# LitLeo/3m-asr-inference

Hardware: AMD Instinct MI355X
Metric: encoder frames/sec, 18Lx32e Conformer-MoE, 206-frame utterance (higher is better)
Workload: dtype f32; 1 GPU; 18-layer 32-expert fp32 (v_mfma_f32_16x16x4_f32), batch=1x206 frames per GPU, all experts local (BASELINE.json configs[1]); layers=18, experts=32, frames=206, batch_per_gpu=1, parallelism=replicas x1, streams_per_gpu=4, hip_graph=True, kernels_per_forward=267, fold_pos_proj=True, routing=balanced, route_mode=staged, packed_rows=False, fork_embed=auto

## Files before the change

### 3m-asr-inference_amd/csrc/engine.hip

```cpp
#include <assert.h>
#include <math.h>
#include <stdlib.h>
#include <string.h>

#include <functional>
#include <memory>
#include <string>
#include <unordered_map>
#include <vector>

#include "../../include/m3asr.h"
#include "common.h"
#include "kernels.h"

namespace m3 {
struct MoeWorkspace {
  int32_t* mapping; int32_t* acc; int32_t* pos; float* slab; size_t bytes;
};
MoeWorkspace carve_moe_workspace(void* base, int S, int E, int D, int F);
}

using namespace m3;

namespace {
// ... 57 lines not shown
  struct Bound {
    int B = 0, T = 0, Tp = 0, S = 0;
    const float* feat = nullptr; const int32_t* feat_len = nullptr; float* logits = nullptr;
    void* ws = nullptr; size_t ws_bytes = 0;
    float* splitk_ws = nullptr; size_t splitk_bytes = 0;
    bool a16 = false;
    bool dma = false;
    bool packed = false;
    bool xn_skipped = false;
    bool lens_in_conv1 = false;
    const float *tail_ln_g = nullptr, *tail_ln_b = nullptr; float tail_ln_eps = 0.f; float* tail_ln_out = nullptr;
    int ep_cap = 0;
    void* sstate = nullptr; int s_hist = 0, s_maxf = 0;
    bool s_slots = false;
    int fork_first = -1, fork_mid = -1, join_at = -1;
    std::shared_ptr<float> pfold;
    std::vector<Stage> stages;
    std::unordered_map<std::string, Buf> buffers;
    int n_kernels = 0;
    hipGraphExec_t graph_exec = nullptr;
    bool graph_valid = false;
    uint64_t last_use = 0;
    bool matches(int b, int t, const float* f, const int32_t* fl, const float* lg, const void* w, size_t wb, int cap,
                 const void* st = nullptr, int hist = 0, int maxf = 0, bool slots = false) const {
      return !stages.empty() && B == b && T == t && feat == f && feat_len == fl && logits == lg && ws == w && ws_bytes == wb &&
             ep_cap == cap && sstate == st && s_hist == hist && s_maxf == maxf && s_slots == slots;
    }
  };
  Bound cur;
  std::vector<Bound> parked;
  uint64_t use_clock = 0;
  int n_captures = 0;
  int ep_capacity = 0;
  hipStream_t side = nullptr;
  hipEvent_t ev_fork = nullptr, ev_join = nullptr;
  std::unordered_map<int, std::weak_ptr<float>> pfold_by_tp;
};

namespace {

struct Switches {
  int gate_index_max_rows;
  bool self_route;
  bool hfuse;
  int router_min_rows;
  bool router_xq;
  bool router_skip_xn;
  bool fused8_adapt;
};
const Switches& switches() {
  static const Switches sw = [] {
    auto num = [](const char* name, int dflt) { const char* v = getenv(name); return v ? atoi(v) : dflt; };
    Switches w;
    w.gate_index_max_rows = num("M3_GATE_INDEX_MAX_ROWS", 512);
    w.self_route = num("M3_SELF_ROUTE", 1) != 0;
    w.hfuse = num("M3_HFUSE", 1) != 0;
    w.router_min_rows = num("M3_ROUTER_MIN_ROWS", 2048);
    w.router_xq = num("M3_ROUTER_XQ", 1) != 0;
    w.router_skip_xn = num("M3_ROUTER_SKIP_XN", 0) != 0;
    w.fused8_adapt = num("M3_FUSED8_ADAPT", 0) != 0;
    return w;
  }();
  return sw;
}

bool lookup(const m3_engine* e, const std::string& name, int64_t numel, const float** out, int dtype = M3_F32) {
  auto it = e->table.find(name);
  if (it == e->table.end()) {
    set_error("engine: weight '%s' missing from the plan", name.c_str());
    return false;
  }
// ... 89 lines not shown
  return true;
}

bool load_sub(const m3_engine* e, const std::string& p, int D, int idim, SubW* s) {
  const int F2 = ((idim - 1) / 2 - 1) / 2;
  GET(s->c1w, p + "conv.0.weight_9c", 9 * (int64_t)D);
  GET(s->c1b, p + "conv.0.bias", D);
  GETW(s->c2w, p + "conv.2.weight_ohwi", 9 * (int64_t)D * D);
  GET(s->c2b, p + "conv.2.bias", D);
  return load_lin(e, p + "out.0.", D, (int64_t)D * F2, true, &s->out);
}
#undef GET
#undef GETW
#undef GETE

inline int sub_len(int t) { return ((t - 3) / 2 + 1 - 3) / 2 + 1; }

struct Carver {
  char* base; size_t off = 0;
  explicit Carver(void* b) : base((char*)b) {}
  template <typename T> T* take(size_t n) {
    T* p = (T*)(base ? base + off : nullptr);
    off += align_up(n * sizeof(T), 256);
    return p;
  }
};

struct Plan {
  int32_t* lens;
  float *c1, *c2, *x, *emb, *h1, *qkv, *pbuf, *ctx, *glu, *dw, *xn, *rl, *eall;
  void* xb;
  int32_t* moe_fs;
  unsigned char* xq; float* xq_scale;
  float* xstats;
  int32_t* gate_idx; float* gate_val;
  void* moe_ws; size_t moe_ws_bytes;
  float* splitk; size_t splitk_bytes;
  float* taps;
  float* pfold;
  int32_t *row0, *pad_of; float* xpad; void* xbpad; float* lpk;
  int32_t *ep_acc, *ep_mapping, *ep_pos, *ep_map_send, *ep_gate_recv, *ep_overflow; float *wire_a, *wire_b; int ep_cap, ep_rows;
  bool fork;
  bool hfuse;
  float *e_c1, *e_c2, *e_x, *e_h1, *e_qkv, *e_ctx, *e_glu, *e_dw, *e_xpad, *e_splitk, *e_xstats; void *e_xb, *e_xbpad;
  size_t bytes;
};

bool use_fork_embed(const m3_engine_config& c, int B, int S) { return c.fork_embed > 0 && !c.debug_taps; }
bool use_packed_rows(const m3_engine_config& c, int B) {
  if (c.packed_rows < 0 || (c.packed_rows == 0 && B <= 1)) return false;
// ... 26 lines not shown
  p.pbuf = cv.take<float>((size_t)Tp * D * (c.num_blocks + c.embed_blocks));
  p.ctx = cv.take<float>((size_t)S * D);
  p.glu = cv.take<float>((size_t)S * D);
  p.dw = cv.take<float>((size_t)S * D);
  p.xn = cv.take<float>((size_t)S * D);
  p.xq = nullptr; p.xq_scale = nullptr; p.moe_fs = nullptr;
  if (c.weight_dtype == M3_FP8) p.moe_fs = cv.take<int32_t>(64);
  if (c.weight_dtype == M3_FP8 && D == 512) {
    p.xq = cv.take<unsigned char>((size_t)S * D);
    p.xq_scale = cv.take<float>((size_t)S);
  }
  p.rl = cv.take<float>((size_t)S * Etot);
  p.eall = cv.take<float>((size_t)S * Etot * c.num_blocks);
  p.gate_idx = cv.take<int32_t>((size_t)c.num_blocks * S);
  p.gate_val = cv.take<float>((size_t)c.num_blocks * S);
  const bool ep = world > 1 || c.ep_stages > 0;
  p.ep_cap = ep ? (ep_capacity > 0 ? ep_capacity : S) : 0;
  p.ep_rows = ep ? world * (p.ep_cap + 1) : 0;
  p.moe_ws_bytes = carve_moe_workspace(nullptr, ep ? p.ep_rows : S, c.num_experts, c.attention_dim, c.hidden_units).bytes;
  p.moe_ws = cv.take<char>(p.moe_ws_bytes * (size_t)(c.debug_taps ? c.num_blocks : 1));
  p.ep_acc = p.ep_mapping = p.ep_pos = p.ep_map_send = p.ep_gate_recv = p.ep_overflow = nullptr; p.wire_a = p.wire_b = nullptr;
  if (ep) {
    p.ep_overflow = cv.take<int32_t>(64);
    p.ep_acc = cv.take<int32_t>((size_t)Etot + 1);
    p.ep_mapping = cv.take<int32_t>(S);
    p.ep_pos = cv.take<int32_t>(S);
    p.ep_map_send = cv.take<int32_t>(S);
    p.ep_gate_recv = cv.take<int32_t>(p.ep_rows);
    p.wire_a = cv.take<float>((size_t)p.ep_rows * c.attention_dim);
    p.wire_b = cv.take<float>((size_t)p.ep_rows * c.attention_dim);
// ... 361 lines not shown
    f.slices = expert_ffn_w16_slices(f.wmode, R, E, D, F);
  }
  return f;
}

static int launch_expert(const ExpertForm& f, const BlockW& w, const float* x, const MoeWorkspace& mw, int R, int E, int D, int F,
                         hipStream_t s, const float* ln_g = nullptr, const float* ln_b = nullptr, float ln_eps = 0.f,
                         const void* xq = nullptr, const float* xq_scale = nullptr, int32_t* fs_dev = nullptr) {
  if (f.wmode >= 2)
    return launch_expert_ffn_w8a8(x, D, mw.pos, mw.acc, R, E, D, F, w.ew1, w.es1, w.eb1, w.ew2, w.es2, 1, w.h_scale, mw.slab, s,
                                  xq, xq_scale, fs_dev);
  if (f.wmode == 1) return launch_expert_ffn_bf16w(x, D, mw.pos, mw.acc, R, E, D, F, w.ew1, w.eb1, w.ew2, 1, mw.slab, s);
  return launch_expert_ffn_f32(x, D, mw.pos, mw.acc, R, E, D, F, w.ew1, w.eb1, w.ew2, 1, mw.slab, ln_g, ln_b, ln_eps, s);
}

static void add_moe_local_expert(m3_engine* e, const MoeLayer& m, const MoeRoute& r, const ExpertForm& f, const Plan& pl) {
  const bool norm = r.norm_in_expert();
  const float* xin = norm ? m.x : m.xn;
  const bool self_route = r.gate == GateForm::InExpert;
  const void* xq = r.use_xq ? pl.xq : nullptr; const float* xqs = r.use_xq ? pl.xq_scale : nullptr;
  int32_t* fs = r.fs_dev ? pl.moe_fs : nullptr;
  add_stage(e, m.pfx + "moe_local.expert", f.launches, [=](hipStream_t s) {
    const BlockW& w = *m.w;
    const float* ln_g = norm ? w.n_ff.g : nullptr; const float* ln_b = norm ? w.n_ff.b : nullptr; const float ln_eps = norm ? m.eps : 0.f;
    if (self_route)
      return launch_expert_route_ffn_f32(xin, m.D, m.rl, m.live_len, m.live_rpb, m.S, m.E, m.D, m.F, w.ew1, w.eb1, w.ew2, 1, w.eb2,
                                         m.mw.slab, m.gidx, m.gval, m.mw.mapping, m.mw.acc, m.mw.pos, s, ln_g, ln_b, ln_eps);
    return launch_expert(f, w, xin, m.mw, m.S, m.E, m.D, m.F, s, ln_g, ln_b, ln_eps, xq, xqs, fs);
  }, stage_info(f.kernel, 1, -1.0, 4.0 * m.D * m.F * m.S));
}

static void add_moe_local_combine(m3_engine* e, const MoeLayer& m, const MoeRoute& r, const ExpertForm& f, const Plan& pl) {
  const bool self_route = r.gate == GateForm::InExpert;
  const int32_t* cmap = self_route ? nullptr : m.mw.mapping;
  const float* cb2 = self_route ? nullptr : m.w->eb2;
  const int32_t* fs = r.fs_dev ? pl.moe_fs : nullptr;
  const double S = m.S, D = m.D;
  add_stage(e, m.pfx + "moe_local.combine", 1, [=](hipStream_t s) {
    const BlockW& w = *m.w;
    return launch_moe_combine(f.rows, fs ? 4 : f.slices, cmap, m.gidx, m.gv, cb2, m.x, 0.5f, w.n_final.g, w.n_final.b, m.eps, m.x,
                              m.S, m.D, s, m.xb_out, m.xstats_out, fs);
  }, stage_info("moe_combine_kernel", 1, S * D * 4 * (f.slices + 2) + (m.xb_out ? 2.0 * S * D : 0.0), S * D * (f.slices + 10)));
}

static void add_moe_ep(m3_engine* e, const MoeLayer& m, const MoeRoute& r, const Plan& pl) {
  const int S = m.S, E = m.E, Etot = m.Etot, D = m.D, F = m.F, world = m.world;
  const int cap = pl.ep_cap, R = pl.ep_rows;
// ... 307 lines not shown
  if (!engine) return;
  if (engine->ev_fork) (void)hipEventDestroy(engine->ev_fork);
  if (engine->ev_join) (void)hipEventDestroy(engine->ev_join);
  if (engine->side) (void)hipStreamDestroy(engine->side);
  if (engine->cur.graph_exec) (void)hipGraphExecDestroy(engine->cur.graph_exec);
  for (auto& b : engine->parked)
    if (b.graph_exec) (void)hipGraphExecDestroy(b.graph_exec);
  delete engine;
}

size_t m3_engine_workspace_size(const m3_engine* engine, int B, int T) {
  if (!engine || B <= 0 || T < 7) return 0;
  return make_plan(engine->cfg, nullptr, B, T, engine->ep_capacity).bytes;
}

static int prepare_impl(m3_engine* e, const float* feat, const int32_t* feat_len, int B, int T, float* logits,
                        void* workspace, size_t workspace_bytes, void* sstate, int s_hist, int s_maxf, bool s_slots = false) {
  M3_REQUIRE(e && feat && feat_len && logits && workspace, "engine_prepare: null argument");
  M3_REQUIRE(B > 0 && T >= 7, "engine_prepare: need B > 0 and T >= 7 frames (got B=%d T=%d)", B, T);
  const m3_engine_config& c = e->cfg;
  const int Tp = sub_len(T);
  M3_REQUIRE(Tp < e->pe_rows, "engine_prepare: T'=%d exceeds the positional table (%lld rows)", Tp,
             (long long)e->pe_rows);
  if (int rc = init_expert_ffn_kernels()) return rc;
  if (int rc = init_expert_ffn_bf16_kernels()) return rc;
  if (int rc = init_expert_ffn_w8_kernels()) return rc;
  if (int rc = init_gemm_bf16_tiled_kernels()) return rc;
  if (int rc = init_expert_ffn_f32_tiled_kernels()) return rc;
  if (int rc = init_expert_ffn_fused_fp8_kernels()) return rc;
  if (int rc = init_gemm_f32_tiled_kernels()) return rc;
// ... 16 lines not shown
          if (e->parked[i].last_use < e->parked[lru].last_use) lru = i;
        if (e->parked[lru].graph_exec) (void)hipGraphExecDestroy(e->parked[lru].graph_exec);
        e->parked.erase(e->parked.begin() + lru);
      }
      e->parked.push_back(std::move(e->cur));
    } else if (e->cur.graph_exec) {
      (void)hipGraphExecDestroy(e->cur.graph_exec);
    }
    e->cur = m3_engine::Bound();
  }
  for (size_t i = 0; i < e->parked.size(); ++i)
    if (e->parked[i].matches(B, T, feat, feat_len, logits, workspace, workspace_bytes, e->ep_capacity, sstate, s_hist, s_maxf, s_slots)) {
      e->cur = std::move(e->parked[i]);
      e->parked.erase(e->parked.begin() + i);
      e->cur.last_use = ++e->use_clock;
      return (int)e->cur.stages.size();
    }
  e->cur.last_use = ++e->use_clock;
  e->cur.B = B; e->cur.T = T; e->cur.Tp = Tp; e->cur.S = B * Tp;
  e->cur.feat = feat; e->cur.feat_len = feat_len; e->cur.logits = logits; e->cur.ws = workspace; e->cur.ws_bytes = workspace_bytes;
  e->cur.ep_cap = e->ep_capacity;
  e->cur.sstate = sstate; e->cur.s_hist = s_hist; e->cur.s_maxf = s_maxf; e->cur.s_slots = s_slots;
  const bool streaming = sstate != nullptr;
  e->cur.stages.clear(); e->cur.buffers.clear(); e->cur.n_kernels = 0; e->cur.graph_valid = false; e->cur.xn_skipped = false;
  e->cur.splitk_ws = pl.splitk; e->cur.splitk_bytes = pl.splitk_bytes;
  {
    GemmParams t;
    t.M = B * Tp; t.N = c.attention_dim; t.K = c.attention_dim; t.w_bf16 = 1;
    e->cur.a16 = c.weight_dtype != M3_F32 && c.bf16_activations >= 0 && !c.debug_taps && c.embed_dim == c.attention_dim &&
                 (c.embed_linear_units % 128) == 0 && (c.hidden_units % 128) == 0 && gemm_bf16w_uses_tiled(t);
  }
  {
    GemmParams t;
    t.M = B * Tp; t.N = c.attention_dim; t.K = c.attention_dim; t.lda = c.attention_dim; t.w_bf16 = 1; t.a_bf16 = 1;
    e->cur.dma = e->cur.a16 && c.attention_dim == 128 * kXbStatParts && gemm_bf16w_uses_dma(t);
  }
  e->cur.packed = use_packed_rows(c, B);
  if (streaming) {
    e->cur.a16 = e->cur.dma = e->cur.packed = false;
// ... 120 lines not shown
    } else
    add_stage(e, "stream.advance", 1, [=](hipStream_t s) { return launch_advance_counter(step, 1, s); },
              stage_info("advance_counter_kernel", 1, 8.0, 0.0, false));
  }
  e->cur.buffers["x"] = Buf{pl.x, (size_t)S * D * 4};
  if (!e->cur.xn_skipped) e->cur.buffers["xn"] = Buf{pl.xn, (size_t)S * D * 4};
  if (pl.xq != nullptr) {
    e->cur.buffers["xq"] = Buf{pl.xq, (size_t)S * D};
    e->cur.buffers["xq_scale"] = Buf{pl.xq_scale, (size_t)S * 4};
  }
  e->cur.buffers["embed"] = Buf{pl.emb, (size_t)S * De * 4};
  if (e->cur.a16) e->cur.buffers["xb"] = Buf{pl.xb, (size_t)S * D * 2};
  e->cur.buffers["lens"] = Buf{pl.lens, (size_t)B * 4};
  if (e->cur.packed) e->cur.buffers["row0"] = Buf{pl.row0, (size_t)(B + 1) * 4};
  if (pl.ep_rows) e->cur.buffers["ep.gate_recv"] = Buf{pl.ep_gate_recv, (size_t)pl.ep_rows * 4};
  e->cur.buffers["router_logits"] = Buf{pl.rl, (size_t)S * c.num_experts * (c.ep_world_size > 0 ? c.ep_world_size : 1) * 4};

  return (int)e->cur.stages.size();
}

int m3_engine_prepare(m3_engine* e, const float* feat, const int32_t* feat_len, int B, int T, float* logits,
                      void* workspace, size_t workspace_bytes) {
  return prepare_impl(e, feat, feat_len, B, T, logits, workspace, workspace_bytes, nullptr, 0, 0);
}

int m3_engine_set_ep_capacity(m3_engine* engine, int rows_per_chunk) {
  M3_REQUIRE(engine != nullptr && rows_per_chunk >= 0, "engine_set_ep_capacity: bad argument");
  engine->ep_capacity = rows_per_chunk;
  return 0;
}
// ... 214 lines not shown
```

### 3m-asr-inference_amd/csrc/kernels.h

```cpp
#pragma once
#include <hip/hip_runtime.h>
#include <stdint.h>

#include "../../include/m3asr.h"

namespace m3 {

enum { ACT_NONE = 0, ACT_RELU = 1, ACT_SILU = 2, ACT_GLU = 3 };
enum { GEMM_A_PLAIN = 0, GEMM_A_CONCAT2 = 1, GEMM_A_CONV3X3S2 = 2 };

struct GemmParams {
  const float* A = nullptr; int lda = 0;
  const float* A2 = nullptr; int lda2 = 0; int K1 = 0;
  const float* W = nullptr;
  int w_bf16 = 0;
  const float* bias = nullptr;
  float* Y = nullptr; int ldy = 0;
  int M = 0, N = 0, K = 0;
  int mode = GEMM_A_PLAIN;
  const float* ln_gamma = nullptr; const float* ln_beta = nullptr; float ln_eps = 0.f;
  const float* ln_wsum = nullptr; const float* ln_wbeta = nullptr;
  int ln_on_a2 = 0;
  float* ln_out = nullptr; int ld_ln_out = 0;
  const int32_t* row_len = nullptr; int rows_per_batch = 0;
// ... 93 lines not shown
int init_expert_ffn_fused_fp8_kernels();
int launch_expert_ffn_fused_fp8(const float* x, int ldx, const int32_t* pos, const int32_t* acc_hist, int S, int E, int D, int F,
                                const void* w1, const float* s1, const float* b1, const void* w2, const float* s2, int w2_sliced,
                                float h_scale, float* ybuf, hipStream_t stream, const void* xq = nullptr, const float* xq_scale = nullptr,
                                int32_t* fs_dev = nullptr);
int launch_quantize_rows_e4m3(const float* x, int ldx, int S, int D, void* xq, float* scale, hipStream_t stream);
bool expert_ffn_w8a8_fused(int S, int E, int D, int F);
int launch_expert_ffn_w8a8(const float* x, int ldx, const int32_t* pos, const int32_t* acc_hist, int S, int E, int D, int F,
                           const void* w1, const float* s1, const float* b1, const void* w2, const float* s2, int w2_sliced,
                           float h_scale, float* slab, hipStream_t stream, const void* xq = nullptr, const float* xq_scale = nullptr,
                           int32_t* fs_dev = nullptr);
int launch_expert_ffn_bf16w_tiled(const float* x, int ldx, const int32_t* pos, const int32_t* acc_hist, int S, int E,
                                  int D, int F, const void* w1, const float* b1, const void* w2, int w2_sliced,
                                  void* hbuf, float* ybuf, hipStream_t stream, const float* b2 = nullptr, float* y_scatter = nullptr);
bool expert_ffn_f32_self_routing(int S, int E);
int launch_expert_route_ffn_f32(const float* x, int ldx, const float* logits, const int32_t* row_len, int rows_per_batch, int S, int E,
                                int D, int F, const float* w1, const float* b1, const float* w2, int w2_sliced, const float* b2,
                                float* slab, int32_t* gate_idx, float* gate_value, int32_t* mapping, int32_t* acc_hist, int32_t* pos,
                                hipStream_t stream, const float* ln_gamma = nullptr, const float* ln_beta = nullptr, float ln_eps = 0.f);
bool expert_ffn_bf16_g256(int S, int E, int D, int F);
int init_expert_gemm_g256_kernels();
int launch_rows_to_bf16(const float* x, int ldx, int S, int D, void* xb, hipStream_t stream);
int launch_expert_ffn_bf16_g256(const void* xb, int ldxb, const int32_t* pos, const int32_t* acc_hist, int S, int E, int D, int F,
                                const void* w1, const float* b1, const void* w2, int w2_sliced, void* hbuf, float* ybuf,
                                hipStream_t stream);
int launch_moe_combine(const float* slab, int n_slices, const int32_t* mapping, const int32_t* gate_idx,
                       const float* gate_value, const float* b2, const float* resid, float alpha,
                       const float* ln_gamma, const float* ln_beta, float ln_eps, float* out, int S, int D,
                       hipStream_t stream, void* out_bf16 = nullptr, float* out_stats = nullptr,
                       const int32_t* n_slices_dev = nullptr);

int launch_layernorm(const float* x, const float* gamma, const float* beta, float eps, float* y, int rows, int D,
                     hipStream_t stream, void* y_bf16 = nullptr, float* y_stats = nullptr, const float* gamma2 = nullptr,
                     const float* beta2 = nullptr, float eps2 = 0.f, float* y2 = nullptr);
// ... 117 lines not shown
```

### 3m-asr-inference_amd/csrc/moe_expert.hip

```cpp
#include "common.h"
#include "kernels.h"
#include "moe_gate.h"

namespace m3 {

struct ExpertRoute {
  const float* logits = nullptr;
  const int32_t* row_len = nullptr; int rows_per_batch = 0;
  int32_t* gate_idx = nullptr; float* gate_value = nullptr;
  int32_t* mapping = nullptr; int32_t* acc_hist = nullptr; int32_t* pos = nullptr;
  const float* b2 = nullptr;
};

template <int MT, bool LNS, int RE = 0>
__global__ __launch_bounds__(64 * (kExpertSlice / 16)) void expert_ffn_f32_kernel(const float* __restrict__ x, int ldx,
                                                             const int32_t* __restrict__ pos,
                                                             const int32_t* __restrict__ acc_hist, int S, int D,
                                                             int F, const float* __restrict__ w1,
                                                             const float* __restrict__ b1,
                                                             const float* __restrict__ w2, int w2_row_stride,
                                                             int w2_slice_stride, float* __restrict__ slab,
                                                             const float* __restrict__ ln_gamma,
                                                             const float* __restrict__ ln_beta, float ln_eps, ExpertRoute rt) {
  extern __shared__ __attribute__((aligned(16))) float lds[];
  const int e = blockIdx.y, slice = blockIdx.x;
  const int lane = threadIdx.x & 63, wave = threadIdx.x >> 6;
  const int col = lane & 15, kq = lane >> 4;

  const int xs_ld = D + 8;
// ... 38 lines not shown
      }
    }
  };
  constexpr int REW = RE > 0 ? RE : 8;
  f32x4 lrow[REW / 4];
  const int rt_r = 64 * wave + lane;
  bool rt_live = false;
  if (RE > 0) {
    rt_live = rt_r < S && (rt.row_len == nullptr || (rt_r % rt.rows_per_batch) < rt.row_len[rt_r / rt.rows_per_batch]);
    const float* lp = rt.logits + (size_t)min(rt_r, S - 1) * RE;
#pragma unroll
    for (int j = 0; j < REW / 4; ++j) lrow[j] = ldg4(lp + 4 * j);
  }
  int row_lo, row_hi;
  __shared__ int32_t route_rows[RE > 0 ? 64 * (kExpertSlice / 16) : 1];
  __shared__ int route_cnt[RE > 0 ? 2 * (kExpertSlice / 16) : 1];
  if (RE > 0) {
    constexpr int NWR = kExpertSlice / 16;
    const int r = rt_r;
    const bool live = rt_live;
    int gi = -1;
    float gv = 0.f;
    gate_top1_regs<REW>(lrow, &gi, &gv, slice == 0);
    if (!live) { gi = -1; gv = 0.f; }
    const unsigned long long mine = __ballot(gi == e), below = __ballot(live && gi < e);
    if (lane == 0) {
      route_cnt[wave] = __popcll(mine);
      route_cnt[NWR + wave] = __popcll(below);
    }
    __syncthreads();
    int off = 0, n_e = 0, acc_e = 0;
#pragma unroll
    for (int w = 0; w < NWR; ++w) {
      if (w < wave) off += route_cnt[w];
      n_e += route_cnt[w];
      acc_e += route_cnt[NWR + w];
    }
    const int rank = off + __popcll(mine & ((1ull << lane) - 1ull));
    if (gi == e) route_rows[rank] = r;
    if (slice == 0) {
// ... 6 lines not shown
        rt.gate_idx[r] = -1;
        rt.gate_value[r] = 0.f;
        if (rt.mapping) rt.mapping[r] = -1;
      }
      if (rt.acc_hist && threadIdx.x == 0) {
        rt.acc_hist[e] = acc_e;
        if (e == RE - 1) rt.acc_hist[RE] = acc_e + n_e;
      }
    }
    row_lo = 0;
    row_hi = n_e;
  } else {
    row_lo = acc_hist[e];
    row_hi = acc_hist[e + 1];
  }
  if (row_hi <= row_lo) return;

  for (int r0 = row_lo + 16 * MT * blockIdx.z; r0 < row_hi; r0 += 16 * MT * gridDim.z) {
    const int nrows = min(16 * MT, row_hi - r0);
    float* slab_base = slab + ((size_t)slice * S + (RE > 0 ? 0 : r0)) * D;

    load_group(0, 0);

    __syncthreads();
    for (int i = wave; i < 16 * MT; i += NWV) {
      float* dst = xs + i * xs_ld;
      if (i < nrows) {
        const float* src = x + (size_t)(RE > 0 ? route_rows[r0 + i] : pos[r0 + i]) * ldx;
        if (LNS) {
          f32x4 v[8];
          float s = 0.f;
#pragma unroll
          for (int j = 0; j < 8; ++j) {
            const int c = lane * 4 + 256 * j;
            const f32x4 t = ldg4(src + min(c, D - 4));
            const bool in = c < D;
            v[j] = f32x4{in ? t[0] : 0.f, in ? t[1] : 0.f, in ? t[2] : 0.f, in ? t[3] : 0.f};
            s += (v[j][0] + v[j][1]) + (v[j][2] + v[j][3]);
          }
          const float mean = wave_sum(s) / (float)D;
          float q = 0.f;
#pragma unroll
          for (int j = 0; j < 8; ++j) {
// ... 94 lines not shown

#pragma unroll
    for (int b = 1; b < NB - 1; ++b)
      if (b < total) load_group(b, b);
    for (int g0 = 0; g0 < total; g0 += NB) {
#pragma unroll
      for (int b = 0; b < NB; ++b) {
        const int g = g0 + b;
        if (g < total) {
          if (g + NB - 1 < total) load_group(g + NB - 1, (b + NB - 1) % NB);
          if (g == g1) transition();
          compute(g, b);
        }
      }
    }
  }
}

int init_expert_ffn_kernels() {
  static PerDeviceOnce once;
  if (once.done()) return 0;
  M3_CHECK_HIP(hipFuncSetAttribute((const void*)expert_ffn_f32_kernel<2, false>, hipFuncAttributeMaxDynamicSharedMemorySize, 160 * 1024));
  M3_CHECK_HIP(hipFuncSetAttribute((const void*)expert_ffn_f32_kernel<4, false>, hipFuncAttributeMaxDynamicSharedMemorySize, 160 * 1024));
  M3_CHECK_HIP(hipFuncSetAttribute((const void*)expert_ffn_f32_kernel<2, true>, hipFuncAttributeMaxDynamicSharedMemorySize, 160 * 1024));
  M3_CHECK_HIP(hipFuncSetAttribute((const void*)expert_ffn_f32_kernel<4, true>, hipFuncAttributeMaxDynamicSharedMemorySize, 160 * 1024));
  once.mark();
  return 0;
}

size_t expert_ffn_slab_bytes(int S, int D, int F) {
// ... 18 lines not shown
  const int w2_row_stride = w2_sliced ? kExpertSlice : F;
  const int w2_slice_stride = w2_sliced ? D * kExpertSlice : kExpertSlice;
  if (int rc = init_expert_ffn_kernels()) return rc;
#define M3_EXPERT_CASE2(MT_, LNS_)                                                                      \
  hipLaunchKernelGGL((expert_ffn_f32_kernel<MT_, LNS_>), grid, dim3(64 * (kExpertSlice / 16)), lds_bytes, stream, x, ldx, pos,    \
                     acc_hist, S, D, F, w1, b1, w2, w2_row_stride, w2_slice_stride, slab, ln_gamma, ln_beta, ln_eps, ExpertRoute())
#define M3_EXPERT_CASE(MT_) do { if (ln_gamma) M3_EXPERT_CASE2(MT_, true); else M3_EXPERT_CASE2(MT_, false); } while (0)
  if (mt == 1) M3_EXPERT_CASE(1); else if (mt == 2) M3_EXPERT_CASE(2); else M3_EXPERT_CASE(4);
#undef M3_EXPERT_CASE
#undef M3_EXPERT_CASE2
  M3_LAUNCH_CHECK();
  return 0;
}

bool expert_ffn_f32_self_routing(int S, int E) { return S >= 1 && S <= 64 * (kExpertSlice / 16) && (E == 8 || E == 16 || E == 32 || E == 64); }

int launch_expert_route_ffn_f32(const float* x, int ldx, const float* logits, const int32_t* row_len, int rows_per_batch, int S, int E,
                                int D, int F, const float* w1, const float* b1, const float* w2, int w2_sliced, const float* b2,
                                float* slab, int32_t* gate_idx, float* gate_value, int32_t* mapping, int32_t* acc_hist, int32_t* pos,
                                hipStream_t stream, const float* ln_gamma, const float* ln_beta, float ln_eps) {
  M3_REQUIRE(expert_ffn_f32_self_routing(S, E), "expert_route_ffn: needs 1 <= S <= %d rows and 8/16/32/64 experts (S=%d E=%d)", 64 * (kExpertSlice / 16), S, E);
  M3_REQUIRE((D & 15) == 0 && D <= 2048 && F % kExpertSlice == 0 && (ldx & 3) == 0, "expert_route_ffn: bad dims D=%d F=%d ldx=%d", D, F, ldx);
  M3_REQUIRE(logits && gate_idx && gate_value && slab, "expert_route_ffn: null pointer");
  M3_REQUIRE(row_len == nullptr || rows_per_batch > 0, "expert_route_ffn: rows_per_batch missing");
  const int mt = S <= 64 ? 1 : 2;
  const size_t lds_bytes = (size_t)16 * mt * ((D + 8) + (kExpertSlice + 8)) * sizeof(float);
  M3_REQUIRE(lds_bytes <= 150 * 1024, "expert_route_ffn: LDS tile of %zu bytes does not fit", lds_bytes);
  static PerDeviceOnce once;
  if (!once.done()) {
#define M3_ROUTE_ATTR(MT_, E_)                                                                                                                            \
  M3_CHECK_HIP(hipFuncSetAttribute((const void*)expert_ffn_f32_kernel<MT_, false, E_>, hipFuncAttributeMaxDynamicSharedMemorySize, 150 * 1024)); \
  M3_CHECK_HIP(hipFuncSetAttribute((const void*)expert_ffn_f32_kernel<MT_, true, E_>, hipFuncAttributeMaxDynamicSharedMemorySize, 150 * 1024))
    M3_ROUTE_ATTR(2, 8); M3_ROUTE_ATTR(2, 16); M3_ROUTE_ATTR(2, 32); M3_ROUTE_ATTR(2, 64);
#undef M3_ROUTE_ATTR
    once.mark();
  }
  ExpertRoute rt;
  rt.logits = logits; rt.row_len = row_len; rt.rows_per_batch = rows_per_batch; rt.gate_idx = gate_idx; rt.gate_value = gate_value;
  rt.mapping = mapping; rt.acc_hist = acc_hist; rt.pos = pos; rt.b2 = b2;
  dim3 grid(F / kExpertSlice, E, 1);
  const int w2_row_stride = w2_sliced ? kExpertSlice : F;
  const int w2_slice_stride = w2_sliced ? D * kExpertSlice : kExpertSlice;
#define M3_ROUTE_CASE(MT_, E_)                                                                                              \
  do {                                                                                                                      \
    if (ln_gamma != nullptr)                                                                                                \
      hipLaunchKernelGGL((expert_ffn_f32_kernel<MT_, true, E_>), grid, dim3(64 * (kExpertSlice / 16)), lds_bytes, stream, x, ldx, \
                         nullptr, nullptr, S, D, F, w1, b1, w2, w2_row_stride, w2_slice_stride, slab, ln_gamma, ln_beta, ln_eps, rt); \
    else                                                                                                                    \
      hipLaunchKernelGGL((expert_ffn_f32_kernel<MT_, false, E_>), grid, dim3(64 * (kExpertSlice / 16)), lds_bytes, stream, x, ldx, \
                         nullptr, nullptr, S, D, F, w1, b1, w2, w2_row_stride, w2_slice_stride, slab, nullptr, nullptr, 0.f, rt); \
  } while (0)
#define M3_ROUTE_E(E_) do { if (mt == 1) M3_ROUTE_CASE(1, E_); else M3_ROUTE_CASE(2, E_); } while (0)
  switch (E) {
    case 8: M3_ROUTE_E(8); break;
    case 16: M3_ROUTE_E(16); break;
    case 32: M3_ROUTE_E(32); break;
    default: M3_ROUTE_E(64); break;
  }
#undef M3_ROUTE_E
#undef M3_ROUTE_CASE
  M3_LAUNCH_CHECK();
  return 0;
}

template <int NV>
__global__ __launch_bounds__(256) void moe_combine_kernel(const float* __restrict__ slab, int n_slices,
                                                          const int32_t* __restrict__ mapping,
                                                          const int32_t* __restrict__ gate_idx,
                                                          const float* __restrict__ gate_value,
                                                          const float* __restrict__ b2,
                                                          const float* resid, float alpha,
                                                          const float* __restrict__ ln_gamma,
                                                          const float* __restrict__ ln_beta, float ln_eps,
                                                          float* out, int S, int D, bf16_t* out_b, float* out_stats,
                                                          const int32_t* __restrict__ n_slices_dev) {
  const int lane = threadIdx.x & 63, wave = threadIdx.x >> 6;
  const int s = blockIdx.x * 4 + wave;
  if (s >= S) return;
  if (n_slices_dev != nullptr) n_slices = min(n_slices, *n_slices_dev);
  const int g = gate_idx ? gate_idx[s] : 0;
  const int m = mapping ? mapping[s] : (g >= 0 ? s : -1);
  const float gate = (m >= 0) ? (gate_value ? gate_value[s] : 1.f) : 0.f;
  f32x4 v[NV];
  float sum = 0.f;
#pragma unroll
  for (int i = 0; i < NV; ++i) {
    const int c = (lane + 64 * i) * 4;
    v[i] = f32x4{0.f, 0.f, 0.f, 0.f};
    if (c < D) {
      f32x4 y = f32x4{0.f, 0.f, 0.f, 0.f};
      constexpr int INF = NV <= 2 ? 16 : 8;
      if (mapping == nullptr) {
        for (int k0 = 0; k0 < n_slices; k0 += INF) {
          f32x4 t[INF];
#pragma unroll
          for (int j = 0; j < INF; ++j)
            t[j] = (k0 + j < n_slices) ? ldg4(slab + ((size_t)(k0 + j) * S + s) * D + c) : f32x4{0.f, 0.f, 0.f, 0.f};
#pragma unroll
          for (int j = 0; j < INF; ++j) y += t[j];
        }
        if (b2) y += ldg4(b2 + (size_t)max(g, 0) * D + c);
        if (m < 0) y = f32x4{0.f, 0.f, 0.f, 0.f};
      } else if (m >= 0) {
        if (b2) y = ldg4(b2 + (size_t)g * D + c);
        for (int k0 = 0; k0 < n_slices; k0 += INF) {
          f32x4 t[INF];
#pragma unroll
          for (int j = 0; j < INF; ++j)
            t[j] = (k0 + j < n_slices) ? ldg4(slab + ((size_t)(k0 + j) * S + m) * D + c) : f32x4{0.f, 0.f, 0.f, 0.f};
#pragma unroll
          for (int j = 0; j < INF; ++j) y += t[j];
        }
      }
      y *= (alpha * gate);
      if (resid) y += ldg4(resid + (size_t)s * D + c);
      v[i] = y;
      sum += (y[0] + y[1]) + (y[2] + y[3]);
    }
  }
  if (ln_gamma) {
    const float mean = wave_sum(sum) / (float)D;
    float q = 0.f;
#pragma unroll
    for (int i = 0; i < NV; ++i) {
      const int c = (lane + 64 * i) * 4;
      if (c < D) {
#pragma unroll
        for (int j = 0; j < 4; ++j) {
          const float d = v[i][j] - mean;
          q += d * d;
        }
      }
    }
    const float rstd = rsqrtf(wave_sum(q) / (float)D + ln_eps);
#pragma unroll
    for (int i = 0; i < NV; ++i) {
      const int c = (lane + 64 * i) * 4;
      if (c < D) {
        const f32x4 ga = ldg4(ln_gamma + c), be = ldg4(ln_beta + c);
#pragma unroll
        for (int j = 0; j < 4; ++j) v[i][j] = (v[i][j] - mean) * rstd * ga[j] + be[j];
      }
    }
  }
  float t1 = 0.f, t2 = 0.f;
#pragma unroll
  for (int i = 0; i < NV; ++i) {
    const int c = (lane + 64 * i) * 4;
    if (c < D) {
      stg4(out + (size_t)s * D + c, v[i]);
      if (out_b != nullptr) {
        bf16x4 h;
#pragma unroll
        for (int j = 0; j < 4; ++j) {
          h[j] = (bf16_t)v[i][j];
          const float f = (float)h[j];
          t1 += f;
          t2 += f * f;
        }
        *reinterpret_cast<bf16x4*>(out_b + (size_t)s * D + c) = h;
      }
    }
  }
  if (out_stats != nullptr) {
    t1 = wave_sum(t1);
    t2 = wave_sum(t2);
    if (lane < 2 * kXbStatParts) out_stats[(size_t)s * 2 * kXbStatParts + lane] = lane == 0 ? t1 : (lane == 1 ? t2 : 0.f);
  }
}

int launch_moe_combine(const float* slab, int n_slices, const int32_t* mapping, const int32_t* gate_idx,
                       const float* gate_value, const float* b2, const float* resid, float alpha,
                       const float* ln_gamma, const float* ln_beta, float ln_eps, float* out, int S, int D,
                       hipStream_t stream, void* out_bf16, float* out_stats, const int32_t* n_slices_dev) {
  M3_REQUIRE((D & 3) == 0 && D <= 2048, "moe_combine: D=%d must be a multiple of 4 (<=2048)", D);
  if (S == 0) return 0;
  const int nv = cdiv(D, 256);
  dim3 grid(cdiv(S, 4));
#define M3_COMBINE_CASE(NV_)                                                                              \
  hipLaunchKernelGGL((moe_combine_kernel<NV_>), grid, dim3(256), 0, stream, slab, n_slices, mapping,     \
                     gate_idx, gate_value, b2, resid, alpha, ln_gamma, ln_beta, ln_eps, out, S, D, (bf16_t*)out_bf16, out_stats, n_slices_dev)
  if (nv <= 1) M3_COMBINE_CASE(1); else if (nv <= 2) M3_COMBINE_CASE(2); else if (nv <= 4) M3_COMBINE_CASE(4); else M3_COMBINE_CASE(8);
#undef M3_COMBINE_CASE
// ... 6 lines not shown
```

Before: 149,000 frames/s.

## Fold MoE combine into self-routing expert FFN via last-block ticket

```diff
diff --git a/3m-asr-inference_amd/csrc/engine.hip b/3m-asr-inference_amd/csrc/engine.hip
--- a/3m-asr-inference_amd/csrc/engine.hip
+++ b/3m-asr-inference_amd/csrc/engine.hip
@@ -95,6 +95,7 @@
     void* sstate = nullptr; int s_hist = 0, s_maxf = 0;
     bool s_slots = false;
     int fork_first = -1, fork_mid = -1, join_at = -1;
+    int32_t* fold_tickets = nullptr;
     std::shared_ptr<float> pfold;
     std::vector<Stage> stages;
     std::unordered_map<std::string, Buf> buffers;
@@ -124,6 +125,7 @@
   int gate_index_max_rows;
   bool self_route;
   bool hfuse;
+  bool fold_combine;
   int router_min_rows;
   bool router_xq;
   bool router_skip_xn;
@@ -136,6 +138,7 @@
     w.gate_index_max_rows = num("M3_GATE_INDEX_MAX_ROWS", 512);
     w.self_route = num("M3_SELF_ROUTE", 1) != 0;
     w.hfuse = num("M3_HFUSE", 1) != 0;
+    w.fold_combine = num("M3_FOLD_COMBINE", 1) != 0;
     w.router_min_rows = num("M3_ROUTER_MIN_ROWS", 2048);
     w.router_xq = num("M3_ROUTER_XQ", 1) != 0;
     w.router_skip_xn = num("M3_ROUTER_SKIP_XN", 0) != 0;
@@ -255,6 +258,8 @@
 #undef GETW
 #undef GETE
 
+constexpr int kFoldTickets = 64;
+
 inline int sub_len(int t) { return ((t - 3) / 2 + 1 - 3) / 2 + 1; }
 
 struct Carver {
@@ -275,6 +280,7 @@
   unsigned char* xq; float* xq_scale;
   float* xstats;
   int32_t* gate_idx; float* gate_val;
+  int32_t* fold_tickets;
   void* moe_ws; size_t moe_ws_bytes;
   float* splitk; size_t splitk_bytes;
   float* taps;
@@ -331,6 +337,7 @@
   p.eall = cv.take<float>((size_t)S * Etot * c.num_blocks);
   p.gate_idx = cv.take<int32_t>((size_t)c.num_blocks * S);
   p.gate_val = cv.take<float>((size_t)c.num_blocks * S);
+  p.fold_tickets = cv.take<int32_t>(kFoldTickets);
   const bool ep = world > 1 || c.ep_stages > 0;
   p.ep_cap = ep ? (ep_capacity > 0 ? ep_capacity : S) : 0;
   p.ep_rows = ep ? world * (p.ep_cap + 1) : 0;
@@ -722,23 +729,37 @@
   return launch_expert_ffn_f32(x, D, mw.pos, mw.acc, R, E, D, F, w.ew1, w.eb1, w.ew2, 1, mw.slab, ln_g, ln_b, ln_eps, s);
 }
 
+static bool fold_moe_combine(const m3_engine_config& c, const MoeLayer& m, const MoeRoute& r, const Plan& pl) {
+  return switches().fold_combine && c.weight_dtype == M3_F32 && r.gate == GateForm::InExpert && !r.ep && !r.fs_dev &&
+         m.xb_out == nullptr && m.xstats_out == nullptr && m.E <= kFoldTickets && expert_ffn_f32_folds_combine(m.D);
+}
+
 static void add_moe_local_expert(m3_engine* e, const MoeLayer& m, const MoeRoute& r, const ExpertForm& f, const Plan& pl) {
   const bool norm = r.norm_in_expert();
   const float* xin = norm ? m.x : m.xn;
   const bool self_route = r.gate == GateForm::InExpert;
+  const bool fold = fold_moe_combine(e->cfg, m, r, pl);
+  int32_t* tickets = pl.fold_tickets;
+  if (fold) e->cur.fold_tickets = tickets;
   const void* xq = r.use_xq ? pl.xq : nullptr; const float* xqs = r.use_xq ? pl.xq_scale : nullptr;
   int32_t* fs = r.fs_dev ? pl.moe_fs : nullptr;
   add_stage(e, m.pfx + "moe_local.expert", f.launches, [=](hipStream_t s) {
     const BlockW& w = *m.w;
     const float* ln_g = norm ? w.n_ff.g : nullptr; const float* ln_b = norm ? w.n_ff.b : nullptr; const float ln_eps = norm ? m.eps : 0.f;
-    if (self_route)
+    if (self_route) {
+      ExpertFold fo;
+      fo.x = m.x; fo.tickets = tickets; fo.gated = m.gv != nullptr; fo.alpha = 0.5f;
+      fo.ln_gamma = w.n_final.g; fo.ln_beta = w.n_final.b; fo.ln_eps = m.eps;
       return launch_expert_route_ffn_f32(xin, m.D, m.rl, m.live_len, m.live_rpb, m.S, m.E, m.D, m.F, w.ew1, w.eb1, w.ew2, 1, w.eb2,
-                                         m.mw.slab, m.gidx, m.gval, m.mw.mapping, m.mw.acc, m.mw.pos, s, ln_g, ln_b, ln_eps);
+                                         m.mw.slab, m.gidx, m.gval, m.mw.mapping, m.mw.acc, m.mw.pos, s, ln_g, ln_b, ln_eps,
+                                         fold ? &fo : nullptr);
+    }
     return launch_expert(f, w, xin, m.mw, m.S, m.E, m.D, m.F, s, ln_g, ln_b, ln_eps, xq, xqs, fs);
-  }, stage_info(f.kernel, 1, -1.0, 4.0 * m.D * m.F * m.S));
+  }, stage_info(f.kernel, 1, -1.0, 4.0 * m.D * m.F * m.S + (fold ? (double)m.S * m.D * (f.slices + 10) : 0.0)));
 }
 
 static void add_moe_local_combine(m3_engine* e, const MoeLayer& m, const MoeRoute& r, const ExpertForm& f, const Plan& pl) {
+  if (fold_moe_combine(e->cfg, m, r, pl)) return;
   const bool self_route = r.gate == GateForm::InExpert;
   const int32_t* cmap = self_route ? nullptr : m.mw.mapping;
   const float* cb2 = self_route ? nullptr : m.w->eb2;
@@ -1076,6 +1097,13 @@
   return make_plan(engine->cfg, nullptr, B, T, engine->ep_capacity).bytes;
 }
 
+static int zero_fold_tickets(int32_t* tickets) {
+  if (tickets == nullptr) return 0;
+  M3_CHECK_HIP(hipMemsetAsync(tickets, 0, kFoldTickets * sizeof(int32_t), nullptr));
+  M3_CHECK_HIP(hipStreamSynchronize(nullptr));
+  return 0;
+}
+
 static int prepare_impl(m3_engine* e, const float* feat, const int32_t* feat_len, int B, int T, float* logits,
                         void* workspace, size_t workspace_bytes, void* sstate, int s_hist, int s_maxf, bool s_slots = false) {
   M3_REQUIRE(e && feat && feat_len && logits && workspace, "engine_prepare: null argument");
@@ -1122,6 +1150,7 @@
       e->cur = std::move(e->parked[i]);
       e->parked.erase(e->parked.begin() + i);
       e->cur.last_use = ++e->use_clock;
+      if (int rc = zero_fold_tickets(e->cur.fold_tickets)) return rc;
       return (int)e->cur.stages.size();
     }
   e->cur.last_use = ++e->use_clock;
@@ -1131,6 +1160,7 @@
   e->cur.sstate = sstate; e->cur.s_hist = s_hist; e->cur.s_maxf = s_maxf; e->cur.s_slots = s_slots;
   const bool streaming = sstate != nullptr;
   e->cur.stages.clear(); e->cur.buffers.clear(); e->cur.n_kernels = 0; e->cur.graph_valid = false; e->cur.xn_skipped = false;
+  e->cur.fold_tickets = nullptr;
   e->cur.splitk_ws = pl.splitk; e->cur.splitk_bytes = pl.splitk_bytes;
   {
     GemmParams t;
@@ -1281,6 +1311,10 @@
   e->cur.buffers["lens"] = Buf{pl.lens, (size_t)B * 4};
   if (e->cur.packed) e->cur.buffers["row0"] = Buf{pl.row0, (size_t)(B + 1) * 4};
   if (pl.ep_rows) e->cur.buffers["ep.gate_recv"] = Buf{pl.ep_gate_recv, (size_t)pl.ep_rows * 4};
+  if (e->cur.fold_tickets != nullptr) {
+    if (int rc = zero_fold_tickets(e->cur.fold_tickets)) return rc;
+    e->cur.buffers["moe_fold.tickets"] = Buf{e->cur.fold_tickets, kFoldTickets * sizeof(int32_t)};
+  }
   e->cur.buffers["router_logits"] = Buf{pl.rl, (size_t)S * c.num_experts * (c.ep_world_size > 0 ? c.ep_world_size : 1) * 4};
 
   return (int)e->cur.stages.size();
diff --git a/3m-asr-inference_amd/csrc/kernels.h b/3m-asr-inference_amd/csrc/kernels.h
--- a/3m-asr-inference_amd/csrc/kernels.h
+++ b/3m-asr-inference_amd/csrc/kernels.h
@@ -131,10 +131,19 @@
                                   int D, int F, const void* w1, const float* b1, const void* w2, int w2_sliced,
                                   void* hbuf, float* ybuf, hipStream_t stream, const float* b2 = nullptr, float* y_scatter = nullptr);
 bool expert_ffn_f32_self_routing(int S, int E);
+struct ExpertFold {
+  float* x = nullptr;
+  int32_t* tickets = nullptr;
+  bool gated = true;
+  float alpha = 1.f;
+  const float* ln_gamma = nullptr; const float* ln_beta = nullptr; float ln_eps = 0.f;
+};
+bool expert_ffn_f32_folds_combine(int D);
 int launch_expert_route_ffn_f32(const float* x, int ldx, const float* logits, const int32_t* row_len, int rows_per_batch, int S, int E,
                                 int D, int F, const float* w1, const float* b1, const float* w2, int w2_sliced, const float* b2,
                                 float* slab, int32_t* gate_idx, float* gate_value, int32_t* mapping, int32_t* acc_hist, int32_t* pos,
-                                hipStream_t stream, const float* ln_gamma = nullptr, const float* ln_beta = nullptr, float ln_eps = 0.f);
+                                hipStream_t stream, const float* ln_gamma = nullptr, const float* ln_beta = nullptr, float ln_eps = 0.f,
+                                const ExpertFold* fold = nullptr);
 bool expert_ffn_bf16_g256(int S, int E, int D, int F);
 int init_expert_gemm_g256_kernels();
 int launch_rows_to_bf16(const float* x, int ldx, int S, int D, void* xb, hipStream_t stream);
diff --git a/3m-asr-inference_amd/csrc/moe_expert.hip b/3m-asr-inference_amd/csrc/moe_expert.hip
--- a/3m-asr-inference_amd/csrc/moe_expert.hip
+++ b/3m-asr-inference_amd/csrc/moe_expert.hip
@@ -3,6 +3,99 @@
 #include "moe_gate.h"
 
 namespace m3 {
+
+template <int NV>
+__device__ __forceinline__ void moe_combine_row(const float* __restrict__ slab, int n_slices, bool direct, int s, int m, int g, float gate,
+                                                const float* __restrict__ b2, const float* resid, float alpha,
+                                                const float* __restrict__ ln_gamma, const float* __restrict__ ln_beta, float ln_eps,
+                                                float* out, int S, int D, bf16_t* out_b, float* out_stats, int lane) {
+  f32x4 v[NV];
+  float sum = 0.f;
+#pragma unroll
+  for (int i = 0; i < NV; ++i) {
+    const int c = (lane + 64 * i) * 4;
+    v[i] = f32x4{0.f, 0.f, 0.f, 0.f};
+    if (c < D) {
+      f32x4 y = f32x4{0.f, 0.f, 0.f, 0.f};
+      constexpr int INF = NV <= 2 ? 16 : 8;
+      if (direct) {
+        for (int k0 = 0; k0 < n_slices; k0 += INF) {
+          f32x4 t[INF];
+#pragma unroll
+          for (int j = 0; j < INF; ++j)
+            t[j] = (k0 + j < n_slices) ? ldg4(slab + ((size_t)(k0 + j) * S + s) * D + c) : f32x4{0.f, 0.f, 0.f, 0.f};
+#pragma unroll
+          for (int j = 0; j < INF; ++j) y += t[j];
+        }
+        if (b2) y += ldg4(b2 + (size_t)max(g, 0) * D + c);
+        if (m < 0) y = f32x4{0.f, 0.f, 0.f, 0.f};
+      } else if (m >= 0) {
+        if (b2) y = ldg4(b2 + (size_t)g * D + c);
+        for (int k0 = 0; k0 < n_slices; k0 += INF) {
+          f32x4 t[INF];
+#pragma unroll
+          for (int j = 0; j < INF; ++j)
+            t[j] = (k0 + j < n_slices) ? ldg4(slab + ((size_t)(k0 + j) * S + m) * D + c) : f32x4{0.f, 0.f, 0.f, 0.f};
+#pragma unroll
+          for (int j = 0; j < INF; ++j) y += t[j];
+        }
+      }
+      y *= (alpha * gate);
+      if (resid) y += ldg4(resid + (size_t)s * D + c);
+      v[i] = y;
+      sum += (y[0] + y[1]) + (y[2] + y[3]);
+    }
+  }
+  if (ln_gamma) {
+    const float mean = wave_sum(sum) / (float)D;
+    float q = 0.f;
+#pragma unroll
+    for (int i = 0; i < NV; ++i) {
+      const int c = (lane + 64 * i) * 4;
+      if (c < D) {
+#pragma unroll
+        for (int j = 0; j < 4; ++j) {
+          const float d = v[i][j] - mean;
+          q += d * d;
+        }
+      }
+    }
+    const float rstd = rsqrtf(wave_sum(q) / (float)D + ln_eps);
+#pragma unroll
+    for (int i = 0; i < NV; ++i) {
+      const int c = (lane + 64 * i) * 4;
+      if (c < D) {
+        const f32x4 ga = ldg4(ln_gamma + c), be = ldg4(ln_beta + c);
+#pragma unroll
+        for (int j = 0; j < 4; ++j) v[i][j] = (v[i][j] - mean) * rstd * ga[j] + be[j];
+      }
+    }
+  }
+  float t1 = 0.f, t2 = 0.f;
+#pragma unroll
+  for (int i = 0; i < NV; ++i) {
+    const int c = (lane + 64 * i) * 4;
+    if (c < D) {
+      stg4(out + (size_t)s * D + c, v[i]);
+      if (out_b != nullptr) {
+        bf16x4 h;
+#pragma unroll
+        for (int j = 0; j < 4; ++j) {
+          h[j] = (bf16_t)v[i][j];
+          const float f = (float)h[j];
+          t1 += f;
+          t2 += f * f;
+        }
+        *reinterpret_cast<bf16x4*>(out_b + (size_t)s * D + c) = h;
+      }
+    }
+  }
+  if (out_stats != nullptr) {
+    t1 = wave_sum(t1);
+    t2 = wave_sum(t2);
+    if (lane < 2 * kXbStatParts) out_stats[(size_t)s * 2 * kXbStatParts + lane] = lane == 0 ? t1 : (lane == 1 ? t2 : 0.f);
+  }
+}
 
 struct ExpertRoute {
   const float* logits = nullptr;
@@ -10,9 +103,14 @@
   int32_t* gate_idx = nullptr; float* gate_value = nullptr;
   int32_t* mapping = nullptr; int32_t* acc_hist = nullptr; int32_t* pos = nullptr;
   const float* b2 = nullptr;
+  float* fold_x = nullptr;
+  int32_t* fold_tickets = nullptr;
+  int fold_gated = 1;
+  float fold_alpha = 1.f;
+  const float* fold_gamma = nullptr; const float* fold_beta = nullptr; float fold_eps = 0.f;
 };
 
-template <int MT, bool LNS, int RE = 0>
+template <int MT, bool LNS, int RE = 0, bool FOLD = false>
 __global__ __launch_bounds__(64 * (kExpertSlice / 16)) void expert_ffn_f32_kernel(const float* __restrict__ x, int ldx,
                                                              const int32_t* __restrict__ pos,
                                                              const int32_t* __restrict__ acc_hist, int S, int D,
@@ -81,7 +179,18 @@
   }
   int row_lo, row_hi;
   __shared__ int32_t route_rows[RE > 0 ? 64 * (kExpertSlice / 16) : 1];
-  __shared__ int route_cnt[RE > 0 ? 2 * (kExpertSlice / 16) : 1];
+  __shared__ int route_cnt[RE > 0 ? 2 * (kExpertSlice / 16) + 1 : 1];
+  static_assert(!FOLD || RE > 0, "the folded combine belongs to the self-routing form");
+  const float* xg = (FOLD && LNS) ? rt.fold_x : x;
+  unsigned long long fold_pad = 0ull;
+  auto fold_pad_rows = [&]() {
+    while (FOLD && fold_pad) {
+      const int r = 64 * wave + __ffsll((long long)fold_pad) - 1;
+      fold_pad &= fold_pad - 1ull;
+      moe_combine_row<2>(slab, (int)gridDim.x, true, r, -1, -1, 0.f, nullptr, rt.fold_x, rt.fold_alpha, rt.fold_gamma, rt.fold_beta,
+                         rt.fold_eps, rt.fold_x, S, D, nullptr, nullptr, lane);
+    }
+  };
   if (RE > 0) {
     constexpr int NWR = kExpertSlice / 16;
     const int r = rt_r;
@@ -91,6 +200,7 @@
     gate_top1_regs<REW>(lrow, &gi, &gv, slice == 0);
     if (!live) { gi = -1; gv = 0.f; }
     const unsigned long long mine = __ballot(gi == e), below = __ballot(live && gi < e);
+    if (FOLD && e == 0 && slice == 0) fold_pad = __ballot(r < S && !live);
     if (lane == 0) {
       route_cnt[wave] = __popcll(mine);
       route_cnt[NWR + wave] = __popcll(below);
@@ -127,7 +237,10 @@
     row_lo = acc_hist[e];
     row_hi = acc_hist[e + 1];
   }
-  if (row_hi <= row_lo) return;
+  if (row_hi <= row_lo) {
+    if (FOLD) fold_pad_rows();
+    return;
+  }
 
   for (int r0 = row_lo + 16 * MT * blockIdx.z; r0 < row_hi; r0 += 16 * MT * gridDim.z) {
     const int nrows = min(16 * MT, row_hi - r0);
@@ -139,7 +252,7 @@
     for (int i = wave; i < 16 * MT; i += NWV) {
       float* dst = xs + i * xs_ld;
       if (i < nrows) {
-        const float* src = x + (size_t)(RE > 0 ? route_rows[r0 + i] : pos[r0 + i]) * ldx;
+        const float* src = xg + (size_t)(RE > 0 ? route_rows[r0 + i] : pos[r0 + i]) * ldx;
         if (LNS) {
           f32x4 v[8];
           float s = 0.f;
@@ -264,6 +377,42 @@
         }
       }
     }
+  }
+
+  if (FOLD) {
+    constexpr int NWR = kExpertSlice / 16;
+    asm volatile("s_waitcnt vmcnt(0)" ::: "memory");
+    __syncthreads();
+    if (threadIdx.x == 0) {
+      __builtin_amdgcn_fence(__ATOMIC_RELEASE, "agent");
+      asm volatile("s_waitcnt vmcnt(0)" ::: "memory");
+      const int ticket = __hip_atomic_fetch_add(rt.fold_tickets + e, 1, __ATOMIC_RELAXED, __HIP_MEMORY_SCOPE_AGENT);
+      const bool last = ticket == (int)gridDim.x - 1;
+      if (last) {
+        __builtin_amdgcn_fence(__ATOMIC_ACQUIRE, "agent");
+        asm volatile("s_waitcnt vmcnt(0)" ::: "memory");
+        __hip_atomic_store(rt.fold_tickets + e, 0, __ATOMIC_RELAXED, __HIP_MEMORY_SCOPE_AGENT);
+      }
+      route_cnt[2 * NWR] = last ? 1 : 0;
+    }
+    __syncthreads();
+    if (route_cnt[2 * NWR]) {
+      for (int i = wave; i < row_hi; i += NWR) {
+        const int r = route_rows[i];
+        float gate = 1.f;
+        if (rt.fold_gated) {
+          f32x4 lr[REW / 4];
+          const float* lp = rt.logits + (size_t)r * RE;
+#pragma unroll
+          for (int j = 0; j < REW / 4; ++j) lr[j] = ldg4(lp + 4 * j);
+          int gi;
+          gate_top1_regs<REW>(lr, &gi, &gate, true);
+        }
+        moe_combine_row<2>(slab, (int)gridDim.x, true, r, r, e, gate, nullptr, rt.fold_x, rt.fold_alpha, rt.fold_gamma, rt.fold_beta,
+                           rt.fold_eps, rt.fold_x, S, D, nullptr, nullptr, lane);
+      }
+    }
+    fold_pad_rows();
   }
 }
 
@@ -312,15 +461,18 @@
 }
 
 bool expert_ffn_f32_self_routing(int S, int E) { return S >= 1 && S <= 64 * (kExpertSlice / 16) && (E == 8 || E == 16 || E == 32 || E == 64); }
+bool expert_ffn_f32_folds_combine(int D) { return D > 256 && D <= 512 && (D & 3) == 0; }
 
 int launch_expert_route_ffn_f32(const float* x, int ldx, const float* logits, const int32_t* row_len, int rows_per_batch, int S, int E,
                                 int D, int F, const float* w1, const float* b1, const float* w2, int w2_sliced, const float* b2,
                                 float* slab, int32_t* gate_idx, float* gate_value, int32_t* mapping, int32_t* acc_hist, int32_t* pos,
-                                hipStream_t stream, const float* ln_gamma, const float* ln_beta, float ln_eps) {
+                                hipStream_t stream, const float* ln_gamma, const float* ln_beta, float ln_eps, const ExpertFold* fold) {
   M3_REQUIRE(expert_ffn_f32_self_routing(S, E), "expert_route_ffn: needs 1 <= S <= %d rows and 8/16/32/64 experts (S=%d E=%d)", 64 * (kExpertSlice / 16), S, E);
   M3_REQUIRE((D & 15) == 0 && D <= 2048 && F % kExpertSlice == 0 && (ldx & 3) == 0, "expert_route_ffn: bad dims D=%d F=%d ldx=%d", D, F, ldx);
   M3_REQUIRE(logits && gate_idx && gate_value && slab, "expert_route_ffn: null pointer");
   M3_REQUIRE(row_len == nullptr || rows_per_batch > 0, "expert_route_ffn: rows_per_batch missing");
+  M3_REQUIRE(fold == nullptr || (expert_ffn_f32_folds_combine(D) && fold->x && fold->tickets),
+             "expert_route_ffn: the folded combine needs 256 < D <= 512, x and the ticket counters (D=%d)", D);
   const int mt = S <= 64 ? 1 : 2;
   const size_t lds_bytes = (size_t)16 * mt * ((D + 8) + (kExpertSlice + 8)) * sizeof(float);
   M3_REQUIRE(lds_bytes <= 150 * 1024, "expert_route_ffn: LDS tile of %zu bytes does not fit", lds_bytes);
@@ -328,7 +480,9 @@
   if (!once.done()) {
 #define M3_ROUTE_ATTR(MT_, E_)                                                                                                                            \
   M3_CHECK_HIP(hipFuncSetAttribute((const void*)expert_ffn_f32_kernel<MT_, false, E_>, hipFuncAttributeMaxDynamicSharedMemorySize, 150 * 1024)); \
-  M3_CHECK_HIP(hipFuncSetAttribute((const void*)expert_ffn_f32_kernel<MT_, true, E_>, hipFuncAttributeMaxDynamicSharedMemorySize, 150 * 1024))
+  M3_CHECK_HIP(hipFuncSetAttribute((const void*)expert_ffn_f32_kernel<MT_, true, E_>, hipFuncAttributeMaxDynamicSharedMemorySize, 150 * 1024)); \
+  M3_CHECK_HIP(hipFuncSetAttribute((const void*)expert_ffn_f32_kernel<MT_, false, E_, true>, hipFuncAttributeMaxDynamicSharedMemorySize, 150 * 1024)); \
+  M3_CHECK_HIP(hipFuncSetAttribute((const void*)expert_ffn_f32_kernel<MT_, true, E_, true>, hipFuncAttributeMaxDynamicSharedMemorySize, 150 * 1024))
     M3_ROUTE_ATTR(2, 8); M3_ROUTE_ATTR(2, 16); M3_ROUTE_ATTR(2, 32); M3_ROUTE_ATTR(2, 64);
 #undef M3_ROUTE_ATTR
     once.mark();
@@ -336,17 +490,24 @@
   ExpertRoute rt;
   rt.logits = logits; rt.row_len = row_len; rt.rows_per_batch = rows_per_batch; rt.gate_idx = gate_idx; rt.gate_value = gate_value;
   rt.mapping = mapping; rt.acc_hist = acc_hist; rt.pos = pos; rt.b2 = b2;
+  if (fold != nullptr) {
+    rt.fold_x = fold->x; rt.fold_tickets = fold->tickets; rt.fold_gated = fold->gated ? 1 : 0; rt.fold_alpha = fold->alpha;
+    rt.fold_gamma = fold->ln_gamma; rt.fold_beta = fold->ln_beta; rt.fold_eps = fold->ln_eps;
+  }
   dim3 grid(F / kExpertSlice, E, 1);
   const int w2_row_stride = w2_sliced ? kExpertSlice : F;
   const int w2_slice_stride = w2_sliced ? D * kExpertSlice : kExpertSlice;
+#define M3_ROUTE_LAUNCH(MT_, LNS_, E_, FOLD_)                                                                                \
+  hipLaunchKernelGGL((expert_ffn_f32_kernel<MT_, LNS_, E_, FOLD_>), grid, dim3(64 * (kExpertSlice / 16)), lds_bytes, stream, x, ldx, \
+                     nullptr, nullptr, S, D, F, w1, b1, w2, w2_row_stride, w2_slice_stride, slab, LNS_ ? ln_gamma : nullptr,      \
+                     LNS_ ? ln_beta : nullptr, LNS_ ? ln_eps : 0.f, rt)
 #define M3_ROUTE_CASE(MT_, E_)                                                                                              \
   do {                                                                                                                      \
-    if (ln_gamma != nullptr)                                                                                                \
-      hipLaunchKernelGGL((expert_ffn_f32_kernel<MT_, true, E_>), grid, dim3(64 * (kExpertSlice / 16)), lds_bytes, stream, x, ldx, \
-                         nullptr, nullptr, S, D, F, w1, b1, w2, w2_row_stride, w2_slice_stride, slab, ln_gamma, ln_beta, ln_eps, rt); \
-    else                                                                                                                    \
-      hipLaunchKernelGGL((expert_ffn_f32_kernel<MT_, false, E_>), grid, dim3(64 * (kExpertSlice / 16)), lds_bytes, stream, x, ldx, \
-                         nullptr, nullptr, S, D, F, w1, b1, w2, w2_row_stride, w2_slice_stride, slab, nullptr, nullptr, 0.f, rt); \
+    if (ln_gamma != nullptr) {                                                                                              \
+      if (fold) M3_ROUTE_LAUNCH(MT_, true, E_, true); else M3_ROUTE_LAUNCH(MT_, true, E_, false);                           \
+    } else {                                                                                                                \
+      if (fold) M3_ROUTE_LAUNCH(MT_, false, E_, true); else M3_ROUTE_LAUNCH(MT_, false, E_, false);                         \
+    }                                                                                                                       \
   } while (0)
 #define M3_ROUTE_E(E_) do { if (mt == 1) M3_ROUTE_CASE(1, E_); else M3_ROUTE_CASE(2, E_); } while (0)
   switch (E) {
@@ -357,6 +518,7 @@
   }
 #undef M3_ROUTE_E
 #undef M3_ROUTE_CASE
+#undef M3_ROUTE_LAUNCH
   M3_LAUNCH_CHECK();
   return 0;
 }
@@ -379,92 +541,8 @@
   const int g = gate_idx ? gate_idx[s] : 0;
   const int m = mapping ? mapping[s] : (g >= 0 ? s : -1);
   const float gate = (m >= 0) ? (gate_value ? gate_value[s] : 1.f) : 0.f;
-  f32x4 v[NV];
-  float sum = 0.f;
-#pragma unroll
-  for (int i = 0; i < NV; ++i) {
-    const int c = (lane + 64 * i) * 4;
-    v[i] = f32x4{0.f, 0.f, 0.f, 0.f};
-    if (c < D) {
-      f32x4 y = f32x4{0.f, 0.f, 0.f, 0.f};
-      constexpr int INF = NV <= 2 ? 16 : 8;
-      if (mapping == nullptr) {
-        for (int k0 = 0; k0 < n_slices; k0 += INF) {
-          f32x4 t[INF];
-#pragma unroll
-          for (int j = 0; j < INF; ++j)
-            t[j] = (k0 + j < n_slices) ? ldg4(slab + ((size_t)(k0 + j) * S + s) * D + c) : f32x4{0.f, 0.f, 0.f, 0.f};
-#pragma unroll
-          for (int j = 0; j < INF; ++j) y += t[j];
-        }
-        if (b2) y += ldg4(b2 + (size_t)max(g, 0) * D + c);
-        if (m < 0) y = f32x4{0.f, 0.f, 0.f, 0.f};
-      } else if (m >= 0) {
-        if (b2) y = ldg4(b2 + (size_t)g * D + c);
-        for (int k0 = 0; k0 < n_slices; k0 += INF) {
-          f32x4 t[INF];
-#pragma unroll
-          for (int j = 0; j < INF; ++j)
-            t[j] = (k0 + j < n_slices) ? ldg4(slab + ((size_t)(k0 + j) * S + m) * D + c) : f32x4{0.f, 0.f, 0.f, 0.f};
-#pragma unroll
-          for (int j = 0; j < INF; ++j) y += t[j];
-        }
-      }
-      y *= (alpha * gate);
-      if (resid) y += ldg4(resid + (size_t)s * D + c);
-      v[i] = y;
-      sum += (y[0] + y[1]) + (y[2] + y[3]);
-    }
-  }
-  if (ln_gamma) {
-    const float mean = wave_sum(sum) / (float)D;
-    float q = 0.f;
-#pragma unroll
-    for (int i = 0; i < NV; ++i) {
-      const int c = (lane + 64 * i) * 4;
-      if (c < D) {
-#pragma unroll
-        for (int j = 0; j < 4; ++j) {
-          const float d = v[i][j] - mean;
-          q += d * d;
-        }
-      }
-    }
-    const float rstd = rsqrtf(wave_sum(q) / (float)D + ln_eps);
-#pragma unroll
-    for (int i = 0; i < NV; ++i) {
-      const int c = (lane + 64 * i) * 4;
-      if (c < D) {
-        const f32x4 ga = ldg4(ln_gamma + c), be = ldg4(ln_beta + c);
-#pragma unroll
-        for (int j = 0; j < 4; ++j) v[i][j] = (v[i][j] - mean) * rstd * ga[j] + be[j];
-      }
-    }
-  }
-  float t1 = 0.f, t2 = 0.f;
-#pragma unroll
-  for (int i = 0; i < NV; ++i) {
-    const int c = (lane + 64 * i) * 4;
-    if (c < D) {
-      stg4(out + (size_t)s * D + c, v[i]);
-      if (out_b != nullptr) {
-        bf16x4 h;
-#pragma unroll
-        for (int j = 0; j < 4; ++j) {
-          h[j] = (bf16_t)v[i][j];
-          const float f = (float)h[j];
-          t1 += f;
-          t2 += f * f;
-        }
-        *reinterpret_cast<bf16x4*>(out_b + (size_t)s * D + c) = h;
-      }
-    }
-  }
-  if (out_stats != nullptr) {
-    t1 = wave_sum(t1);
-    t2 = wave_sum(t2);
-    if (lane < 2 * kXbStatParts) out_stats[(size_t)s * 2 * kXbStatParts + lane] = lane == 0 ? t1 : (lane == 1 ? t2 : 0.f);
-  }
+  moe_combine_row<NV>(slab, n_slices, mapping == nullptr, s, m, g, gate, b2, resid, alpha, ln_gamma, ln_beta, ln_eps, out, S, D, out_b,
+                      out_stats, lane);
 }
 
 int launch_moe_combine(const float* slab, int n_slices, const int32_t* mapping, const int32_t* gate_idx,
```

Result: slower. 129,300 frames/s (-13.2%).
